# nerfstudio-project/gsplat

Hardware: AMD Instinct MI355X
Metric: Mpixels/s fwd+bwd @1M Gaussians/1080p (higher is better)
Workload: dtype f32; 1 GPU; c3: 1M synthetic Gaussians, 1x1920x1080, SH deg 3, 16x16 tiles, fwd+bwd; gaussians_per_gpu=1000000, cameras_per_gpu=1, packed=False, parallelism=single

## Files before the change

gsplat_amd/csrc/bitonic64.hpp:

```cpp
#pragma once
#include "common.hpp"

namespace gsx {

constexpr uint64_t kBtPadInt = ~0ull;
constexpr uint64_t kBtPadF64 = 0x7FF0000000000000ull;

__device__ __forceinline__ int bt_phys(int i) { return i + (i >> 3); }
__device__ __forceinline__ int bt_off(int b, int lj)
{
    const int sb = b << lj;
    return sb + (sb >> 3);
}
__device__ __forceinline__ bool bt_key_is_odd(uint32_t depth_bits)
{
    return (depth_bits - 0x00100000u) >= (0x7FF00000u - 0x00100000u);
}

__device__ __forceinline__ void bt_cmpx_int(uint64_t &x, uint64_t &y, bool up)
{
    const bool sw     = (x > y) == up;
    const uint64_t lo = sw ? y : x, hi = sw ? x : y;
    x = lo;
    y = hi;
}
__device__ __forceinline__ void bt_cmpx_int_up(uint64_t &x, uint64_t &y)
{
    const bool sw    = x > y;
    const uint64_t t = sw ? y : x;
    y                = sw ? x : y;
    x                = t;
}

template <int G, int NT>
__device__ __forceinline__ void bt_group_int(uint64_t *s, int P, int lk, int lj, int tid)
{
    constexpr int R = 1 << G;
    for (int t = tid; t < (P >> G); t += NT) {
        const int i = ((t >> lj) << (lj + G)) | (t & ((1 << lj) - 1));
        const uint32_t m32 = 0u - (((uint32_t)i >> lk) & 1u);
        const uint64_t m   = ((uint64_t)m32 << 32) | m32;
        uint64_t *p        = s + bt_phys(i);
        uint64_t e[R];
#pragma unroll
        for (int b = 0; b < R; ++b) e[b] = p[bt_off(b, lj)] ^ m;
#pragma unroll
        for (int q = G - 1; q >= 0; --q)
#pragma unroll
            for (int b = 0; b < R; ++b)
                if (!(b & (1 << q))) bt_cmpx_int_up(e[b], e[b | (1 << q)]);
#pragma unroll
        for (int b = 0; b < R; ++b) p[bt_off(b, lj)] = e[b] ^ m;
    }
}

template <int NT, typename Sync>
__device__ __forceinline__ void bt_sort_int(uint64_t *s, int lp, int tid, Sync &&SYNC)
{
    const int P = 1 << lp;
    for (int t = tid; t < (P >> 3); t += NT) {
        uint64_t *p = s + 9 * t;
        uint64_t e[8];
#pragma unroll
        for (int b = 0; b < 8; ++b) e[b] = p[b];
#pragma unroll
        for (int lk = 1; lk <= 3; ++lk)
#pragma unroll
            for (int q = lk - 1; q >= 0; --q)
#pragma unroll
                for (int b = 0; b < 8; ++b)
                    if (!(b & (1 << q))) {
                        const bool up = lk < 3 ? ((b & (1 << lk)) == 0) : ((t & 1) == 0);
                        bt_cmpx_int(e[b], e[b | (1 << q)], up);
                    }
#pragma unroll
        for (int b = 0; b < 8; ++b) p[b] = e[b];
    }
    SYNC();
    for (int lk = 4; lk <= lp; ++lk) {
        for (int top = lk - 1; top >= 0;) {
            const int gsz = top + 1 < 3 ? top + 1 : 3;
            const int lj  = top - gsz + 1;
            if (gsz == 3) bt_group_int<3, NT>(s, P, lk, lj, tid);
            else if (gsz == 2) bt_group_int<2, NT>(s, P, lk, lj, tid);
            else bt_group_int<1, NT>(s, P, lk, lj, tid);
            SYNC();
            top -= gsz;
        }
    }
}

__device__ __forceinline__ void bt_minmax(double &x, double &y)
{
    double lo, hi;
    asm("v_min_f64 %0, %1, %2" : "=v"(lo) : "v"(x), "v"(y));
    asm("v_max_f64 %0, %1, %2" : "=v"(hi) : "v"(x), "v"(y));
    x = lo;
    y = hi;
}
__device__ __forceinline__ double bt_as_f64(uint64_t w) { return __builtin_bit_cast(double, w); }
__device__ __forceinline__ uint64_t bt_as_u64(double d) { return __builtin_bit_cast(uint64_t, d); }

template <int G, int NT>
__device__ __forceinline__ void bt_group_f64(uint64_t *s, int P, int lk, int lj, int tid)
{
    constexpr int R = 1 << G;
    for (int t = tid; t < (P >> G); t += NT) {
        const int i = ((t >> lj) << (lj + G)) | (t & ((1 << lj) - 1));
        const uint64_t neg = (uint64_t)(((uint32_t)i >> lk) & 1u) << 63;
        uint64_t *p        = s + bt_phys(i);
        double e[R];
#pragma unroll
        for (int b = 0; b < R; ++b) e[b] = bt_as_f64(p[bt_off(b, lj)] ^ neg);
#pragma unroll
        for (int q = G - 1; q >= 0; --q)
#pragma unroll
            for (int b = 0; b < R; ++b)
                if (!(b & (1 << q))) bt_minmax(e[b], e[b | (1 << q)]);
#pragma unroll
        for (int b = 0; b < R; ++b) p[bt_off(b, lj)] = bt_as_u64(e[b]) ^ neg;
    }
}

template <int NT, typename Sync>
__device__ __forceinline__ void bt_sort_f64(uint64_t *s, int lp, int tid, Sync &&SYNC)
{
    const int P = 1 << lp;
    for (int t = tid; t < (P >> 3); t += NT) {
        uint64_t *p = s + 9 * t;
        double e[8];
#pragma unroll
        for (int b = 0; b < 8; ++b) e[b] = bt_as_f64(p[b]);
#pragma unroll
        for (int lk = 1; lk <= 2; ++lk)
#pragma unroll
            for (int q = lk - 1; q >= 0; --q)
#pragma unroll
                for (int b = 0; b < 8; ++b)
                    if (!(b & (1 << q))) {
                        if ((b & (1 << lk)) == 0) bt_minmax(e[b], e[b | (1 << q)]);
                        else bt_minmax(e[b | (1 << q)], e[b]);
                    }
        const uint64_t neg = (uint64_t)((uint32_t)t & 1u) << 63;
#pragma unroll
        for (int b = 0; b < 8; ++b) e[b] = bt_as_f64(bt_as_u64(e[b]) ^ neg);
#pragma unroll
        for (int q = 2; q >= 0; --q)
#pragma unroll
            for (int b = 0; b < 8; ++b)
                if (!(b & (1 << q))) bt_minmax(e[b], e[b | (1 << q)]);
#pragma unroll
        for (int b = 0; b < 8; ++b) p[b] = bt_as_u64(e[b]) ^ neg;
    }
    SYNC();
    for (int lk = 4; lk <= lp; ++lk) {
        for (int top = lk - 1; top >= 0;) {
            const int gsz = top + 1 < 3 ? top + 1 : 3;
            const int lj  = top - gsz + 1;
            if (gsz == 3) bt_group_f64<3, NT>(s, P, lk, lj, tid);
            else if (gsz == 2) bt_group_f64<2, NT>(s, P, lk, lj, tid);
            else bt_group_f64<1, NT>(s, P, lk, lj, tid);
            SYNC();
            top -= gsz;
        }
    }
}

bool bitonic_f64_enabled();

}
```

gsplat_amd/csrc/isect_binned.hip:

```cpp
#include "isect_binwalk.hpp"
#include "bitonic64.hpp"
#include "isect_fused.hpp"
#include <cstdlib>
#include <mutex>
#include <new>

namespace gsx {

constexpr int kRowThreads     = 1024;
constexpr int kBnThreads      = 256;
constexpr int kBnMaxBins      = 16384;
constexpr uint32_t kBnMaxTiles = 36864;

struct BinHeader {
    int32_t overflow;
    int32_t big_count;
    int32_t b_done;
    int32_t pad[5];
};

struct BinGeom {
    int64_t rows, rows_per_image, cap_entries;
    uint32_t n_images, cpi, rpc, n_chunks;
    uint32_t tile_size, tile_w, tile_h, n_tiles;
    uint32_t bw, bh, bins_x, bins_y, n_bins, n_bins_total, tile_bits;
    uint32_t kx, ky;
    int32_t skew_cap;
    int32_t skew_ratio;
};

struct BinBuffers {
    BinHeader *hdr;
    int32_t *table;
    int32_t *bin_count;
    int32_t *unit_count;
    uint4 *unit_rec;
    uint32_t *unit_row;
    int32_t *bin_start;
    uint4 *row_rec;
    uint2 *e_pair;
    uint16_t *e_mask;
    int32_t *tile_count;
    int32_t *big_list;
};

struct BinArgs {
    BinGeom g;
    BinBuffers b;
    const float *means2d;
    const int32_t *radii;
    const float *depths;
    const float *conics;
    const float *opacities;
    const uint8_t *tile_mask;
    int32_t *tiles_per_gauss;
    int32_t *isect_offsets;
    int64_t *n_isects;
    int64_t *max_tile_len;
    uint64_t *keys_out;
    int32_t *vals_out;
    uint2 *bucketed;
    uint32_t sort_int;
};

__device__ __forceinline__ void bn_chunk_rows(const BinGeom &g, uint32_t chunk, int64_t &lo, int64_t &hi, uint32_t &img)
{
    img                = chunk / g.cpi;
    const uint32_t sub = chunk % g.cpi;
    lo                 = (int64_t)img * g.rows_per_image + (int64_t)sub * g.rpc;
    hi                 = min(lo + (int64_t)g.rpc, (int64_t)(img + 1) * g.rows_per_image);
}

struct BnRow {
    float mx, my, rx, ry, A, B, C, op;
};
__device__ __forceinline__ BnRow bn_load_row(const BinArgs &a, int64_t r, bool has_conic)
{
    BnRow q;
    const int2 rad = reinterpret_cast<const int2 *>(a.radii)[r];
// ... 257 lines not shown
    int32_t v[kCsPer];
    int32_t sum = 0;
#pragma unroll
    for (int i = 0; i < kCsPer; ++i) {
        const uint32_t r = r0 + (uint32_t)i;
        v[i]             = (live && r < r1) ? col[(int64_t)r * n_cols] : 0;
    }
#pragma unroll
    for (int i = 0; i < kCsPer; ++i) sum += v[i];
    s_seg[seg][lane_c] = sum;
    __syncthreads();
    int32_t run = 0;
    for (uint32_t k = 0; k < seg; ++k) run += s_seg[k][lane_c];
    if (live) {
#pragma unroll
        for (int i = 0; i < kCsPer; ++i) {
            const uint32_t r = r0 + (uint32_t)i;
            if (r < r1) col[(int64_t)r * n_cols] = run;
            run += v[i];
        }
        if (seg == kCsSegs2 - 1) a.b.bin_count[(int64_t)img * n_cols + c] = run;
    }
    __syncthreads();
    if (threadIdx.x == 0)
        s_last = __hip_atomic_fetch_add(&a.b.hdr->b_done, 1, __ATOMIC_RELEASE, __HIP_MEMORY_SCOPE_AGENT) == (int32_t)gridDim.x - 1;
    __syncthreads();
    if (!s_last) return;
    __builtin_amdgcn_fence(__ATOMIC_ACQUIRE, "agent");
    const int64_t n = block_scan_i32_1024(a.b.bin_count, a.b.bin_start, g.n_bins_total, s_part, &s_max);
    int32_t um = 0;
    for (uint32_t i = threadIdx.x; i < g.n_chunks; i += kCsCols * kCsSegs2) um = max(um, a.b.unit_count[i]);
    um = wave_max_i32(um);
    if ((threadIdx.x & 63u) == 0) s_umax[threadIdx.x >> 6] = um;
    __syncthreads();
    if (threadIdx.x == 0) {
        for (int w = 1; w < 16; ++w) um = max(um, s_umax[w]);
        const int64_t mx    = s_max;
        const bool lopsided = g.skew_ratio > 0 && mx * (int64_t)g.n_bins_total > (int64_t)g.skew_ratio * n && mx > 256;
        a.b.bin_start[g.n_bins_total] = (int32_t)min(n, (int64_t)INT32_MAX);
        a.b.hdr->overflow = (n > g.cap_entries || um > (int32_t)kUnitCap || (g.skew_cap > 0 && mx > g.skew_cap) || lopsided) ? 1 : 0;
    }
}

template <bool FIXED>
__device__ __forceinline__ void bn_deal(const BinArgs &a, const BinShape<FIXED> &sh, const uint4 &rec, uint32_t row, int32_t *s_cur)
{
    const uint32_t bx0 = rec.z & 255u, by0 = (rec.z >> 8) & 255u;
    const uint64_t M   = ((uint64_t)rec.y << 32) | rec.x;
    for (uint32_t used = rec.z >> 18; used;) {
        const uint32_t k = (uint32_t)__builtin_ctz(used);
        used &= used - 1u;
        const uint32_t i = k % sh.kx, j = k / sh.kx;
        const int32_t slot = atomicAdd(&s_cur[(by0 + j) * a.g.bins_x + bx0 + i], 1);
        a.b.e_pair[slot] = make_uint2(rec.w, row);
        a.b.e_mask[slot] = (uint16_t)rec_bin_mask(M, sh, i, j);
    }
}

template <bool FIXED>
__global__ void __launch_bounds__(kRowThreads) bin_scatter_kernel(const BinArgs a)
{
    extern __shared__ int32_t s_cur[];
    const BinGeom &g = a.g;
    const BinShape<FIXED> sh(g);
    const uint32_t per_xcd = gridDim.x / 8u;
    const uint32_t chunk   = (blockIdx.x % 8u) * per_xcd + blockIdx.x / 8u;
    if (chunk >= g.n_chunks) return;
    int64_t lo, hi;
    uint32_t img;
    bn_chunk_rows(g, chunk, lo, hi, img);
    constexpr int kU = 2;
    uint4 rec[kU];
#pragma unroll
    for (int u = 0; u < kU; ++u) {
        const int64_t r = lo + u * kRowThreads + threadIdx.x;
        rec[u]          = r < hi ? a.b.row_rec[r] : make_uint4(0u, 0u, 0u, 0u);
    }
    const int32_t *start = a.b.bin_start + (int64_t)img * g.n_bins;
    const int32_t *pre   = a.b.table + (int64_t)chunk * g.n_bins;
    for (uint32_t i = threadIdx.x; i < g.n_bins; i += kRowThreads) s_cur[i] = start[i] + pre[i];
    const int32_t n_units = min(a.b.unit_count[chunk], (int32_t)kUnitCap);
    if (a.b.hdr->overflow) return;
    __syncthreads();
    for (int64_t base = lo; base < hi; base += kU * kRowThreads) {
#pragma unroll
        for (int u = 0; u < kU; ++u) {
            const int64_t r = base + u * kRowThreads + threadIdx.x;
            if (base != lo) rec[u] = r < hi ? a.b.row_rec[r] : make_uint4(0u, 0u, 0u, 0u);
            if (((rec[u].z >> 16) & 3u) == kRecSmall) bn_deal(a, sh, rec[u], (uint32_t)r, s_cur);
        }
    }
    for (int32_t k = (int32_t)threadIdx.x; k < n_units; k += kRowThreads)
        bn_deal(a, sh, a.b.unit_rec[(size_t)chunk * kUnitCap + k], a.b.unit_row[(size_t)chunk * kUnitCap + k], s_cur);
}

__global__ void __launch_bounds__(kBnThreads) bin_tiles_kernel(const BinArgs a)
{
    __shared__ int32_t s_cnt[16];
    const BinGeom &g = a.g;
    if (a.b.hdr->overflow) return;
    const uint32_t bin = blockIdx.x;
    const int32_t e0 = a.b.bin_start[bin], e1 = a.b.bin_start[bin + 1];
    const int lane = (int)(threadIdx.x & 63u);
    const int n_bits = (int)(g.bw * g.bh);
    if (threadIdx.x < 16) s_cnt[threadIdx.x] = 0;
    __syncthreads();
    int32_t mine = 0;
    constexpr int kU = 8;
    for (int32_t base = e0; base < e1; base += kBnThreads * kU) {
        uint32_t m[kU];
#pragma unroll
        for (int u = 0; u < kU; ++u) {
            const int32_t e = base + u * kBnThreads + (int32_t)threadIdx.x;
            m[u]            = e < e1 ? (uint32_t)a.b.e_mask[e] : 0u;
        }
#pragma unroll
        for (int u = 0; u < kU; ++u) {
            if (base + u * kBnThreads >= e1) break;
            for (int t = 0; t < n_bits; ++t) {
                const uint64_t b = __builtin_amdgcn_ballot_w64((m[u] >> t) & 1u);
                if (lane == t) mine += (int32_t)__popcll(b);
            }
        }
    }
    if (lane < n_bits && mine) atomicAdd(&s_cnt[lane], mine);
    __syncthreads();
    if ((int)threadIdx.x < n_bits) {
        const uint32_t img = bin / g.n_bins, lb = bin % g.n_bins;
        const uint32_t tx = (lb % g.bins_x) * g.bw + threadIdx.x % g.bw, ty = (lb / g.bins_x) * g.bh + threadIdx.x / g.bw;
        if (tx < g.tile_w && ty < g.tile_h) a.b.tile_count[(size_t)img * g.n_tiles + (size_t)ty * g.tile_w + tx] = s_cnt[threadIdx.x];
    }
}

__global__ void __launch_bounds__(1024) tile_plan_kernel(const BinArgs a)
{
    __shared__ int64_t s_part[16];
    __shared__ int32_t s_max;
    const BinGeom &g = a.g;
    if (a.b.hdr->overflow) {
        if (threadIdx.x == 0) {
            __threadfence_system();
            *a.n_isects = GSX_ISECT_RETRY;
        }
        return;
    }
    const uint32_t nt   = g.n_images * g.n_tiles;
    const int64_t total = block_scan_i32_1024(a.b.tile_count, a.isect_offsets, nt, s_part, a.max_tile_len ? &s_max : nullptr);
    if (threadIdx.x == 0) {
        if (a.max_tile_len) *a.max_tile_len = (int64_t)s_max;
        __threadfence_system();
        *a.n_isects = total;
    }
}

constexpr int kArenaPerWave = 544;

__host__ __device__ __forceinline__ int bn_list_words(int n, int &head)
{
    head = 0;
    if (n <= 0) return 0;
    int P = 64;
    while (P < n) P <<= 1;
    const int H = P >> 1;
    if (H >= 256 && n - H <= (H >> 2)) {
        head = H;
        return H + ((n - H + 7) & ~7);
    }
// ... 34 lines not shown
        } else {
            for (int i = lane; i < Pt; i += 64) {
                const uint64_t tv = sw[bt_phys(i)];
                sw[bt_phys(i)]    = keys[i];
                if (i < T) sw[bt_phys(H + i)] = tv;
            }
            lp = 31 - __builtin_clz((unsigned)H);
        }
        wave_lds_sync();
        if (as_int) bt_sort_int<64>(sw, lp, lane, [] { wave_lds_sync(); });
        else bt_sort_f64<64>(sw, lp, lane, [] { wave_lds_sync(); });
    }
    if (H == 0) {
        for (int i = lane; i < n; i += 64) {
            const uint64_t w = sw[bt_phys(i)];
            keys[i]          = hi | (w >> 32);
            vals[i]          = (int32_t)(uint32_t)w;
        }
        return;
    }
    for (int i0 = 0; i0 < H; i0 += 256) {
        uint64_t w[4];
        int r[4];
#pragma unroll
        for (int k = 0; k < 4; ++k) w[k] = sw[bt_phys(i0 + 64 * k + lane)];
        bn_rank4(sw, H, T, w, r);
#pragma unroll
        for (int k = 0; k < 4; ++k) {
            const int pos = i0 + 64 * k + lane + r[k];
            keys[pos]     = hi | (w[k] >> 32);
            vals[pos]     = (int32_t)(uint32_t)w[k];
        }
    }
    for (int j0 = 0; j0 < T; j0 += 256) {
        uint64_t w[4];
        int r[4];
#pragma unroll
        for (int k = 0; k < 4; ++k) {
            const int j = j0 + 64 * k + lane;
            w[k]        = j < T ? sw[bt_phys(H + j)] : 0ull;
        }
        bn_rank4(sw, 0, H, w, r);
#pragma unroll
        for (int k = 0; k < 4; ++k) {
            const int j = j0 + 64 * k + lane;
            if (j < T) {
                keys[j + r[k]] = hi | (w[k] >> 32);
                vals[j + r[k]] = (int32_t)(uint32_t)w[k];
            }
        }
    }
}

__global__ void __launch_bounds__(1024) __attribute__((amdgpu_waves_per_eu(8, 8))) bin_sort_kernel(const BinArgs a)
{
    extern __shared__ __attribute__((aligned(16))) unsigned char smem_raw[];
    const BinGeom &g = a.g;
    const int n_bits = (int)(g.bw * g.bh), n_thr = n_bits * 64;
    const int arena_words = kArenaPerWave * n_bits;
    uint64_t *s_arena = reinterpret_cast<uint64_t *>(smem_raw);
    __shared__ int32_t s_tcnt[16], s_goff[16], s_base[16], s_batch[16], s_cur[16], s_nbatch, s_n;
    __shared__ uint32_t s_odd;
    __shared__ uint64_t s_hi[16];
    const uint32_t bin = blockIdx.x;
    const int32_t e0 = a.b.bin_start[bin], e1 = a.b.bin_start[bin + 1];
    if (e0 == e1) return;
    const uint32_t img = bin / g.n_bins, lb = bin % g.n_bins;
    const uint32_t tx0 = (lb % g.bins_x) * g.bw, ty0 = (lb / g.bins_x) * g.bh;
    const int lane = (int)(threadIdx.x & 63u);
    const int wave = __builtin_amdgcn_readfirstlane((int)(threadIdx.x >> 6));
    if ((int)threadIdx.x < 16) {
        const int t       = (int)threadIdx.x;
        const uint32_t tx = tx0 + (uint32_t)t % g.bw, ty = ty0 + (uint32_t)t / g.bw;
        const bool in     = t < n_bits && tx < g.tile_w && ty < g.tile_h;
        const size_t gid  = (size_t)img * g.n_tiles + (size_t)ty * g.tile_w + tx;
        const int n       = in ? a.b.tile_count[gid] : 0;
        s_tcnt[t]         = n;
        s_goff[t]         = in ? a.isect_offsets[gid] : 0;
        s_hi[t]           = in ? ((((uint64_t)img << g.tile_bits) | ((uint64_t)ty * g.tile_w + tx)) << 32) : 0ull;
        int head;
        int P = bn_list_words(n, head);
        const bool big = P > arena_words;
        if (big) P = 0;
        int batch = 0, used = 0, my_batch = n > 0 ? 0 : -1, my_base = 0;
        for (int k = 0; k < 16; ++k) {
            const int Pk = __shfl(P, k, 16);
            if (Pk == 0) continue;
            if (used + Pk > arena_words) { ++batch; used = 0; }
            if (k == t) { my_batch = batch; my_base = used + (used >> 3); }
            used += Pk;
        }
        s_batch[t] = big ? -2 : my_batch;
        s_base[t]  = my_base;
        if (t == 15) s_nbatch = batch + 1;
    }
    __syncthreads();
    const int n_batch = s_nbatch;
    for (int b = 0; b < n_batch; ++b) {
        if (threadIdx.x < 16) s_cur[threadIdx.x] = 0;
        if (threadIdx.x == 16) s_odd = a.sort_int ? 0xFFFFu : 0u;
        const uint32_t bmask = (uint32_t)__builtin_amdgcn_ballot_w64(lane < n_bits && s_batch[lane & 15] == b);
        __syncthreads();
        for (int32_t e = e0 + (int32_t)threadIdx.x; e < e1; e += n_thr) {
            uint32_t m = (uint32_t)a.b.e_mask[e] & bmask;
            if (m == 0u) continue;
            const uint2 pr     = a.b.e_pair[e];
            const uint64_t key = ((uint64_t)pr.x << 32) | pr.y;
            if (bt_key_is_odd(pr.x)) atomicOr(&s_odd, m);
            while (m) {
                const int t = __builtin_ctz(m);
                m &= m - 1u;
                const int32_t pos = atomicAdd(&s_cur[t], 1);
                s_arena[s_base[t] + bt_phys(pos)] = key;
            }
        }
        __syncthreads();
        if (wave < n_bits && s_batch[wave] == b) {
            uint64_t *sw = s_arena + __builtin_amdgcn_readfirstlane(s_base[wave]);
            const int n  = __builtin_amdgcn_readfirstlane(s_tcnt[wave]);
            const bool as_int = (__builtin_amdgcn_readfirstlane((int)s_odd) >> wave) & 1;
            const int64_t off = __builtin_amdgcn_readfirstlane(s_goff[wave]);
            const uint64_t hi = (uint64_t)(uint32_t)__builtin_amdgcn_readfirstlane((int)(s_hi[wave] >> 32)) << 32;
            int head;
            bn_list_words(n, head);
            bn_sort_list(sw, n, head, as_int, lane, a.keys_out + off, a.vals_out + off, hi);
        }
        __syncthreads();
    }
    for (int t = 0; t < n_bits; ++t) {
        if (s_batch[t] != -2) continue;
        if (threadIdx.x == 0) s_n = 0;
        __syncthreads();
        const int64_t off      = s_goff[t];
        const uint64_t lt_mask = (lane == 0) ? 0ull : (~0ull >> (64 - lane));
        for (int32_t base = e0; base < e1; base += n_thr) {
            const int32_t e    = base + (int32_t)threadIdx.x;
            const bool has     = e < e1 && (((uint32_t)a.b.e_mask[e] >> t) & 1u);
            const uint64_t bal = __builtin_amdgcn_ballot_w64(has);
            if (bal == 0ull) continue;
            const int first = (int)__builtin_ctzll(bal);
            int32_t wbase   = 0;
            if (lane == first) wbase = atomicAdd(&s_n, (int32_t)__popcll(bal));
            wbase = __builtin_amdgcn_readlane(wbase, first);
            if (has) a.bucketed[off + wbase + (int32_t)__popcll(bal & lt_mask)] = a.b.e_pair[e];
        }
        if (threadIdx.x == 0) {
            const uint32_t tx = tx0 + (uint32_t)t % g.bw, ty = ty0 + (uint32_t)t / g.bw;
            a.b.big_list[atomicAdd(&a.b.hdr->big_count, 1)] = (int32_t)(img * g.n_tiles + ty * g.tile_w + tx);
        }
        __syncthreads();
    }
}

static int64_t align256(int64_t x) { return (x + 255) & ~(int64_t)255; }
static uint32_t bits_for(uint64_t count)
{
    uint32_t b = 0;
    if (count <= 1) return 0;
    uint64_t v = count - 1;
    while (v) { ++b; v >>= 1; }
    return b;
}

static void bin_dims(uint32_t &bw, uint32_t &bh)
{
    bw = 4; bh = 2;
    if (const char *e = getenv("GSX_ISECT_BIN")) {
        unsigned w = 0, h = 0;
        if (sscanf(e, "%ux%u", &w, &h) == 2 && w >= 1 && h >= 1 && w * h <= 16) { bw = w; bh = h; }
    }
}

static bool bin_geometry(BinGeom &g, int64_t rows, uint32_t n_images, uint32_t tile_size, uint32_t tile_w, uint32_t tile_h,
                         int64_t cap_entries)
{
    g = BinGeom{};
    g.rows = rows; g.n_images = n_images ? n_images : 1;
    g.rows_per_image = rows / g.n_images;
    bin_dims(g.bw, g.bh);
    g.tile_size = tile_size; g.tile_w = tile_w; g.tile_h = tile_h; g.n_tiles = tile_w * tile_h;
    g.bins_x = (tile_w + g.bw - 1) / g.bw; g.bins_y = (tile_h + g.bh - 1) / g.bh;
    g.kx = 2; g.ky = g.bw * g.bh <= 8 ? 4 : 2;
    g.n_bins = g.bins_x * g.bins_y; g.n_bins_total = g.n_bins * g.n_images;
    g.tile_bits = bits_for(g.n_tiles);
    const int64_t max_cpi = 1024 / g.n_images > 0 ? 1024 / g.n_images : 1;
    int64_t cpi = (g.rows_per_image + 2047) / 2048;
    {
        const int64_t per_image = (256 + (int64_t)g.n_images - 1) / (int64_t)g.n_images;
        const int64_t floor_cpi = g.rows_per_image / 1024 < per_image ? g.rows_per_image / 1024 : per_image;
        if (cpi < floor_cpi) cpi = floor_cpi;
    }
    if (cpi < 1) cpi = 1;
    if (cpi > max_cpi) cpi = max_cpi;
    g.cpi = (uint32_t)cpi;
    g.rpc = (uint32_t)((g.rows_per_image + cpi - 1) / cpi);
    if (g.rpc == 0) g.rpc = 1;
    g.n_chunks    = g.cpi * g.n_images;
    g.cap_entries = cap_entries;
    return g.n_bins_total <= (uint32_t)kBnMaxBins && (uint64_t)g.n_images * g.n_tiles <= kBnMaxTiles && rows < (1ll << 28)
           && g.bins_x <= 256 && g.bins_y <= 256;
}

static int64_t bin_cap_entries(int64_t rows) { return 4 * rows + 262144; }

static int64_t bin_layout(const BinGeom &g, unsigned char *base, BinBuffers *b)
{
    unsigned char *p = base;
    auto take = [&](int64_t bytes) {
        unsigned char *q = p;
        p += align256(bytes);
        return q;
    };
    BinBuffers t{};
    t.hdr        = reinterpret_cast<BinHeader *>(take(sizeof(BinHeader)));
    t.table      = reinterpret_cast<int32_t *>(take((int64_t)g.n_chunks * g.n_bins * 4));
    t.bin_count  = reinterpret_cast<int32_t *>(take((int64_t)g.n_bins_total * 4));
    t.unit_count = reinterpret_cast<int32_t *>(take((int64_t)g.n_chunks * 4));
    t.unit_rec   = reinterpret_cast<uint4 *>(take((int64_t)g.n_chunks * kUnitCap * 16));
    t.unit_row   = reinterpret_cast<uint32_t *>(take((int64_t)g.n_chunks * kUnitCap * 4));
    t.bin_start  = reinterpret_cast<int32_t *>(take(((int64_t)g.n_bins_total + 1) * 4));
    t.row_rec    = reinterpret_cast<uint4 *>(take(g.rows * 16));
    t.e_pair     = reinterpret_cast<uint2 *>(take(g.cap_entries * 8));
    t.e_mask     = reinterpret_cast<uint16_t *>(take(g.cap_entries * 2));
    t.tile_count = reinterpret_cast<int32_t *>(take((int64_t)g.n_images * g.n_tiles * 4));
    t.big_list   = reinterpret_cast<int32_t *>(take((int64_t)g.n_images * g.n_tiles * 4));
    if (b) *b = t;
    return (int64_t)(p - base);
}

}

using namespace gsx;

namespace {
struct RetryNote { uint64_t key; int left; };
struct PathMemory {
    std::mutex mu;
    RetryNote notes[16] = {};
    uint32_t next = 0;
};
thread_local PathMemory t_default_memory;
thread_local PathMemory *t_current_memory = nullptr;
PathMemory &current_memory() { return t_current_memory ? *t_current_memory : t_default_memory; }
uint64_t retry_key(int64_t rows, uint32_t n_images, uint32_t tile_w, uint32_t tile_h)
{
    return ((uint64_t)(rows >> 16) << 40) ^ ((uint64_t)n_images << 32) ^ ((uint64_t)tile_w << 16) ^ (uint64_t)tile_h ^ (1ull << 63);
}
bool retried_recently(int64_t rows, uint32_t n_images, uint32_t tile_w, uint32_t tile_h, bool consume)
{
    const uint64_t key = retry_key(rows, n_images, tile_w, tile_h);
    PathMemory &m = current_memory();
// ... 82 lines not shown
                "%s: %u images x %u x %u tiles not supported", fn, n_images, tile_w, tile_h);
    a.sort_int = bitonic_f64_enabled() ? 0u : 1u;
    {
        const char *force = getenv("GSX_ISECT_PATH");
        a.g.skew_cap = (force && force[0] == 'b') ? 0 : (int32_t)(kArenaPerWave * (int)(a.g.bw * a.g.bh) * 3 / 4);
        a.g.skew_ratio = (force && force[0] == 'b') ? 0 : 4;
    }
    unsigned char *base = reinterpret_cast<unsigned char *>((reinterpret_cast<uintptr_t>(ws) + 255) & ~(uintptr_t)255);
    if (ws == nullptr || (base - reinterpret_cast<unsigned char *>(ws)) + bin_layout(a.g, base, &a.b) > ws_bytes) {
        set_last_error("%s: count workspace too small", fn);
        return GSX_ERR_WORKSPACE;
    }
    return GSX_OK;
}

extern "C" int gsx_isect_binned_count(const float *means2d, const int32_t *radii, const float *depths, const float *conics,
                                      const float *opacities, const uint8_t *tile_mask, int64_t rows, uint32_t n_images,
                                      uint32_t tile_size, uint32_t tile_w, uint32_t tile_h, int32_t *tiles_per_gauss,
                                      int32_t *isect_offsets, int64_t *n_isects, int64_t *max_tile_len, void *count_workspace,
                                      int64_t count_workspace_bytes, void *stream)
{
    hipStream_t s = (hipStream_t)stream;
    const uint32_t n_bins = n_images * tile_w * tile_h;
    GSX_REQUIRE(isect_offsets && n_isects, "gsx_isect_binned_count: null output");
    if (rows == 0) {
        if (max_tile_len && hipMemsetAsync(max_tile_len, 0, 8, s) != hipSuccess) return check_launch("isect_binned_count memset");
        if (hipMemsetAsync(isect_offsets, 0, (size_t)n_bins * 4, s) != hipSuccess
            || hipMemsetAsync(n_isects, 0, 8, s) != hipSuccess) {
            set_last_error("gsx_isect_binned_count: memset failed");
            return GSX_ERR_LAUNCH;
        }
        return GSX_OK;
    }
    GSX_REQUIRE(means2d && radii && depths, "gsx_isect_binned_count: null pointer");
    BinArgs a{};
    int rc = binned_setup("gsx_isect_binned_count", a, rows, n_images, tile_size, tile_w, tile_h, count_workspace,
                          count_workspace_bytes);
    if (rc != GSX_OK) return rc;
    a.means2d = means2d; a.radii = radii; a.depths = depths; a.conics = conics; a.opacities = opacities;
    a.tile_mask = tile_mask; a.tiles_per_gauss = tiles_per_gauss; a.isect_offsets = isect_offsets; a.n_isects = n_isects;
    a.max_tile_len = max_tile_len;
    const size_t bins_lds = (size_t)a.g.n_bins * sizeof(int32_t);
    const bool fixed      = a.g.bw == 4 && a.g.bh == 2 && a.g.kx == 2 && a.g.ky == 4;
    static PerDeviceOnce once;
    if (once.first()) {
        (void)hipFuncSetAttribute((const void *)bin_rect_kernel<true>, hipFuncAttributeMaxDynamicSharedMemorySize, 64 * 1024);
        (void)hipFuncSetAttribute((const void *)bin_rect_kernel<false>, hipFuncAttributeMaxDynamicSharedMemorySize, 64 * 1024);
    }
    if (fixed) bin_rect_kernel<true><<<dim3(a.g.n_chunks), dim3(kRowThreads), bins_lds, s>>>(a);
    else bin_rect_kernel<false><<<dim3(a.g.n_chunks), dim3(kRowThreads), bins_lds, s>>>(a);
    const uint32_t col_groups = (a.g.n_bins + kCsCols - 1) / kCsCols;
    bin_colscan_kernel<<<dim3(col_groups * a.g.n_images), dim3(kCsCols * kCsSegs2), 0, s>>>(a, col_groups);
    const uint32_t d_grid = (a.g.n_chunks + 7u) / 8u * 8u;
    if (fixed) bin_scatter_kernel<true><<<dim3(d_grid), dim3(kRowThreads), bins_lds, s>>>(a);
    else bin_scatter_kernel<false><<<dim3(d_grid), dim3(kRowThreads), bins_lds, s>>>(a);
    bin_tiles_kernel<<<dim3(a.g.n_bins_total), dim3(kBnThreads), 0, s>>>(a);
    tile_plan_kernel<<<dim3(1), dim3(1024), 0, s>>>(a);
    return check_launch("isect_binned_count");
}

extern "C" int gsx_isect_binned_emit_sort(int64_t rows, uint32_t n_images, uint32_t tile_size, uint32_t tile_w,
                                          uint32_t tile_h, void *count_workspace, int64_t count_workspace_bytes,
                                          const int32_t *isect_offsets, int64_t n_isects, int64_t longest_list,
                                          int64_t *isect_ids_sorted, int32_t *flatten_ids_sorted, void *workspace,
                                          int64_t workspace_bytes, void *stream)
{
    GSX_REQUIRE(n_isects >= 0 && n_isects < (1ll << 31), "gsx_isect_binned_emit_sort: n_isects out of range");
    if (n_isects == 0 || rows == 0) return GSX_OK;
    GSX_REQUIRE(isect_offsets && isect_ids_sorted && flatten_ids_sorted, "gsx_isect_binned_emit_sort: null pointer");
    hipStream_t s = (hipStream_t)stream;
    BinArgs a{};
    int rc = binned_setup("gsx_isect_binned_emit_sort", a, rows, n_images, tile_size, tile_w, tile_h, count_workspace,
                          count_workspace_bytes);
    if (rc != GSX_OK) return rc;
    if (workspace == nullptr || workspace_bytes < gsx_isect_binned_emit_workspace_bytes(n_isects)) {
        set_last_error("gsx_isect_binned_emit_sort: workspace too small");
        return GSX_ERR_WORKSPACE;
    }
    unsigned char *p = reinterpret_cast<unsigned char *>((reinterpret_cast<uintptr_t>(workspace) + 255) & ~(uintptr_t)255);
    a.bucketed = reinterpret_cast<uint2 *>(p); p += align256(n_isects * 8);
    uint2 *scratch = reinterpret_cast<uint2 *>(p);
    a.isect_offsets = const_cast<int32_t *>(isect_offsets);
    a.keys_out = reinterpret_cast<uint64_t *>(isect_ids_sorted);
    a.vals_out = flatten_ids_sorted;
    const int n_bits = (int)(a.g.bw * a.g.bh);
    const size_t sort_lds = (size_t)(kArenaPerWave * n_bits) * 9;
    static PerDeviceOnce once;
    if (once.first())
        (void)hipFuncSetAttribute((const void *)bin_sort_kernel, hipFuncAttributeMaxDynamicSharedMemorySize, 112 * 1024);
    bin_sort_kernel<<<dim3(a.g.n_bins_total), dim3(64 * n_bits), sort_lds, s>>>(a);
    rc = check_launch("isect_binned_emit");
    if (rc != GSX_OK) return rc;
    TileSortArgs t{};
    t.n = n_isects; t.n_tiles = a.g.n_tiles; t.tile_bits = a.g.tile_bits; t.n_bins = a.g.n_images * a.g.n_tiles;
    t.n_chunks = 1;
    t.table_scanned = const_cast<int32_t *>(isect_offsets);
    t.bucketed = a.bucketed; t.scratch = scratch;
    t.big_count = &a.b.hdr->big_count; t.big_list = a.b.big_list;
    t.keys_out = a.keys_out; t.vals_out = a.vals_out;
    if (longest_list > 0 && longest_list <= (int64_t)(kArenaPerWave * n_bits) / 2) return GSX_OK;
    return launch_big_tile_sort(t, s);
}
```

gsplat_amd/csrc/isect_binwalk.hpp:

```cpp
#pragma once
#include "isect_walk.hpp"

namespace gsx {

struct WalkPrep {
    int x0, y0, x1, y1;
    bool any;
    bool ellipse, alongY;
    float B, coeff, disc, t, pu, pv, bmin_u, bmax_u, bmin_v, bmax_v, u_at_vmin, u_at_vmax;
};

__host__ __device__ __forceinline__ WalkPrep walk_prepare(float mx, float my, float rx, float ry, bool has_conic, float A,
                                                          float B, float C, float opacity, uint32_t tile_size,
                                                          uint32_t tile_w, uint32_t tile_h)
{
    WalkPrep p;
    p.any = false; p.ellipse = has_conic; p.alongY = false;
    p.x0 = p.y0 = p.x1 = p.y1 = 0;
    p.B = p.coeff = p.disc = p.t = p.pu = p.pv = p.bmin_u = p.bmax_u = p.bmin_v = p.bmax_v = p.u_at_vmin = p.u_at_vmax = 0.0f;
    const float ts     = (float)tile_size;
    const bool ts_pow2 = (tile_size & (tile_size - 1u)) == 0u;
    const float ts_inv = 1.0f / ts;
    auto div_ts        = [&](float x) { return ts_pow2 ? x * ts_inv : x / ts; };
    if (has_conic) {
// ... 84 lines not shown
        if (tv1 > cv1) tv1 = cv1;
        span(p.alongY, u, tv0, tv1);
        lo_lo   = hi_lo;
        lo_hi   = hi_hi;
        line_lo = line_hi;
    }
}

template <typename Emit>
__host__ __device__ __forceinline__ int32_t walk_clipped(const WalkPrep &p, uint32_t tile_size, int cx0, int cy0, int cx1,
                                                         int cy1, Emit &&emit)
{
    int32_t count = 0;
    walk_clipped_spans(p, tile_size, cx0, cy0, cx1, cy1, [&](bool alongY, int u, int tv0, int tv1) {
        for (int v = tv0; v < tv1; ++v) {
            if (alongY) emit(v, u);
            else emit(u, v);
            ++count;
        }
    });
    return count;
}

__host__ __device__ __forceinline__ uint64_t low_bits64(uint32_t n) { return n >= 64u ? ~0ull : ((1ull << n) - 1ull); }

__host__ __device__ __forceinline__ uint64_t block_mask(const WalkPrep &p, uint32_t tile_size, uint32_t tile_w, int cx0, int cy0,
                                                        int cx1, int cy1, uint32_t W, uint64_t col, const uint8_t *tmask)
{
    uint64_t M = 0;
    walk_clipped_spans(p, tile_size, cx0, cy0, cx1, cy1, [&](bool alongY, int uu, int tv0, int tv1) {
        if (tv1 <= tv0) return;
        if (alongY)
            M |= (low_bits64((uint32_t)(tv1 - cx0)) ^ low_bits64((uint32_t)(tv0 - cx0))) << ((uint32_t)(uu - cy0) * W);
        else
            M |= (col & (low_bits64((uint32_t)(tv1 - cy0) * W) ^ low_bits64((uint32_t)(tv0 - cy0) * W))) << (uu - cx0);
    });
    if (tmask)
        for (uint64_t left = M; left;) {
            const int b = __builtin_ctzll(left);
            left &= left - 1ull;
            if (!tmask[(size_t)(cy0 + b / (int)W) * tile_w + (size_t)(cx0 + b % (int)W)]) M &= ~(1ull << b);
        }
    return M;
}

__host__ __device__ __forceinline__ uint32_t block_bin_mask(uint64_t M, uint32_t bw, uint32_t bh, uint32_t kx, uint32_t i, uint32_t j)
{
    const uint32_t W = kx * bw, row_bits = (1u << bw) - 1u;
    uint32_t m = 0;
    for (uint32_t y = 0; y < bh; ++y) m |= ((uint32_t)(M >> ((j * bh + y) * W + i * bw)) & row_bits) << (y * bw);
    return m;
}

}
```

Baseline: 2633 Mpixels/s.

## Pack bin entries into one 64-bit word and sort each bin once

For the fixed 4x2-tile bin geometry, the scatter kernel now packs depth, per-image row and an 8-bit tile mask into one 64-bit word instead of writing separate pair and mask arrays. A new per-bin kernel loads a whole bin into LDS, bitonic-sorts it once, with per-wave sub-sorts followed by block-wide merge steps, and then deals the sorted entries out to the 8 tiles with ballots. This replaces the old path that re-gathered and sorted per tile. The old sort kernel still runs as a fallback for large bins, and the extra launch plus the 24-bit row limit add complexity.

```diff
diff --git a/gsplat_amd/csrc/bitonic64.hpp b/gsplat_amd/csrc/bitonic64.hpp
--- a/gsplat_amd/csrc/bitonic64.hpp
+++ b/gsplat_amd/csrc/bitonic64.hpp
@@ -33,11 +33,11 @@
 }
 
 template <int G, int NT>
-__device__ __forceinline__ void bt_group_int(uint64_t *s, int P, int lk, int lj, int tid)
+__device__ __forceinline__ void bt_group_int(uint64_t *s, int P, int lk, int lj, int tid, int ibase = 0)
 {
     constexpr int R = 1 << G;
     for (int t = tid; t < (P >> G); t += NT) {
-        const int i = ((t >> lj) << (lj + G)) | (t & ((1 << lj) - 1));
+        const int i = ibase + (((t >> lj) << (lj + G)) | (t & ((1 << lj) - 1)));
         const uint32_t m32 = 0u - (((uint32_t)i >> lk) & 1u);
         const uint64_t m   = ((uint64_t)m32 << 32) | m32;
         uint64_t *p        = s + bt_phys(i);
@@ -54,10 +54,9 @@
     }
 }
 
-template <int NT, typename Sync>
-__device__ __forceinline__ void bt_sort_int(uint64_t *s, int lp, int tid, Sync &&SYNC)
+template <int NT>
+__device__ __forceinline__ void bt_head_int(uint64_t *s, int P, int tid)
 {
-    const int P = 1 << lp;
     for (int t = tid; t < (P >> 3); t += NT) {
         uint64_t *p = s + 9 * t;
         uint64_t e[8];
@@ -76,18 +75,27 @@
 #pragma unroll
         for (int b = 0; b < 8; ++b) p[b] = e[b];
     }
+}
+template <int NT, typename Sync>
+__device__ __forceinline__ void bt_phase_int(uint64_t *s, int P, int lk, int top, int tid, int ibase, Sync &&SYNC)
+{
+    while (top >= 0) {
+        const int gsz = top + 1 < 3 ? top + 1 : 3;
+        const int lj  = top - gsz + 1;
+        if (gsz == 3) bt_group_int<3, NT>(s, P, lk, lj, tid, ibase);
+        else if (gsz == 2) bt_group_int<2, NT>(s, P, lk, lj, tid, ibase);
+        else bt_group_int<1, NT>(s, P, lk, lj, tid, ibase);
+        SYNC();
+        top -= gsz;
+    }
+}
+template <int NT, typename Sync>
+__device__ __forceinline__ void bt_sort_int(uint64_t *s, int lp, int tid, Sync &&SYNC)
+{
+    const int P = 1 << lp;
+    bt_head_int<NT>(s, P, tid);
     SYNC();
-    for (int lk = 4; lk <= lp; ++lk) {
-        for (int top = lk - 1; top >= 0;) {
-            const int gsz = top + 1 < 3 ? top + 1 : 3;
-            const int lj  = top - gsz + 1;
-            if (gsz == 3) bt_group_int<3, NT>(s, P, lk, lj, tid);
-            else if (gsz == 2) bt_group_int<2, NT>(s, P, lk, lj, tid);
-            else bt_group_int<1, NT>(s, P, lk, lj, tid);
-            SYNC();
-            top -= gsz;
-        }
-    }
+    for (int lk = 4; lk <= lp; ++lk) bt_phase_int<NT>(s, P, lk, lk - 1, tid, 0, SYNC);
 }
 
 __device__ __forceinline__ void bt_minmax(double &x, double &y)
@@ -102,11 +110,11 @@
 __device__ __forceinline__ uint64_t bt_as_u64(double d) { return __builtin_bit_cast(uint64_t, d); }
 
 template <int G, int NT>
-__device__ __forceinline__ void bt_group_f64(uint64_t *s, int P, int lk, int lj, int tid)
+__device__ __forceinline__ void bt_group_f64(uint64_t *s, int P, int lk, int lj, int tid, int ibase = 0)
 {
     constexpr int R = 1 << G;
     for (int t = tid; t < (P >> G); t += NT) {
-        const int i = ((t >> lj) << (lj + G)) | (t & ((1 << lj) - 1));
+        const int i = ibase + (((t >> lj) << (lj + G)) | (t & ((1 << lj) - 1)));
         const uint64_t neg = (uint64_t)(((uint32_t)i >> lk) & 1u) << 63;
         uint64_t *p        = s + bt_phys(i);
         double e[R];
@@ -122,10 +130,9 @@
     }
 }
 
-template <int NT, typename Sync>
-__device__ __forceinline__ void bt_sort_f64(uint64_t *s, int lp, int tid, Sync &&SYNC)
+template <int NT>
+__device__ __forceinline__ void bt_head_f64(uint64_t *s, int P, int tid)
 {
-    const int P = 1 << lp;
     for (int t = tid; t < (P >> 3); t += NT) {
         uint64_t *p = s + 9 * t;
         double e[8];
@@ -152,18 +159,27 @@
 #pragma unroll
         for (int b = 0; b < 8; ++b) p[b] = bt_as_u64(e[b]) ^ neg;
     }
+}
+template <int NT, typename Sync>
+__device__ __forceinline__ void bt_phase_f64(uint64_t *s, int P, int lk, int top, int tid, int ibase, Sync &&SYNC)
+{
+    while (top >= 0) {
+        const int gsz = top + 1 < 3 ? top + 1 : 3;
+        const int lj  = top - gsz + 1;
+        if (gsz == 3) bt_group_f64<3, NT>(s, P, lk, lj, tid, ibase);
+        else if (gsz == 2) bt_group_f64<2, NT>(s, P, lk, lj, tid, ibase);
+        else bt_group_f64<1, NT>(s, P, lk, lj, tid, ibase);
+        SYNC();
+        top -= gsz;
+    }
+}
+template <int NT, typename Sync>
+__device__ __forceinline__ void bt_sort_f64(uint64_t *s, int lp, int tid, Sync &&SYNC)
+{
+    const int P = 1 << lp;
+    bt_head_f64<NT>(s, P, tid);
     SYNC();
-    for (int lk = 4; lk <= lp; ++lk) {
-        for (int top = lk - 1; top >= 0;) {
-            const int gsz = top + 1 < 3 ? top + 1 : 3;
-            const int lj  = top - gsz + 1;
-            if (gsz == 3) bt_group_f64<3, NT>(s, P, lk, lj, tid);
-            else if (gsz == 2) bt_group_f64<2, NT>(s, P, lk, lj, tid);
-            else bt_group_f64<1, NT>(s, P, lk, lj, tid);
-            SYNC();
-            top -= gsz;
-        }
-    }
+    for (int lk = 4; lk <= lp; ++lk) bt_phase_f64<NT>(s, P, lk, lk - 1, tid, 0, SYNC);
 }
 
 bool bitonic_f64_enabled();
diff --git a/gsplat_amd/csrc/isect_binned.hip b/gsplat_amd/csrc/isect_binned.hip
--- a/gsplat_amd/csrc/isect_binned.hip
+++ b/gsplat_amd/csrc/isect_binned.hip
@@ -25,6 +25,7 @@
     uint32_t tile_size, tile_w, tile_h, n_tiles;
     uint32_t bw, bh, bins_x, bins_y, n_bins, n_bins_total, tile_bits;
     uint32_t kx, ky;
+    uint32_t word;
     int32_t skew_cap;
     int32_t skew_ratio;
 };
@@ -388,8 +389,12 @@
         used &= used - 1u;
         const uint32_t i = k % sh.kx, j = k / sh.kx;
         const int32_t slot = atomicAdd(&s_cur[(by0 + j) * a.g.bins_x + bx0 + i], 1);
-        a.b.e_pair[slot] = make_uint2(rec.w, row);
-        a.b.e_mask[slot] = (uint16_t)rec_bin_mask(M, sh, i, j);
+        if (FIXED) {
+            reinterpret_cast<uint64_t *>(a.b.e_pair)[slot] = bin_entry_pack(rec.w, row, rec_bin_mask(M, sh, i, j));
+        } else {
+            a.b.e_pair[slot] = make_uint2(rec.w, row);
+            a.b.e_mask[slot] = (uint16_t)rec_bin_mask(M, sh, i, j);
+        }
     }
 }
 
@@ -416,6 +421,7 @@
     const int32_t *pre   = a.b.table + (int64_t)chunk * g.n_bins;
     for (uint32_t i = threadIdx.x; i < g.n_bins; i += kRowThreads) s_cur[i] = start[i] + pre[i];
     const int32_t n_units = min(a.b.unit_count[chunk], (int32_t)kUnitCap);
+    const uint32_t row0   = FIXED ? (uint32_t)((int64_t)img * g.rows_per_image) : 0u;
     if (a.b.hdr->overflow) return;
     __syncthreads();
     for (int64_t base = lo; base < hi; base += kU * kRowThreads) {
@@ -423,11 +429,11 @@
         for (int u = 0; u < kU; ++u) {
             const int64_t r = base + u * kRowThreads + threadIdx.x;
             if (base != lo) rec[u] = r < hi ? a.b.row_rec[r] : make_uint4(0u, 0u, 0u, 0u);
-            if (((rec[u].z >> 16) & 3u) == kRecSmall) bn_deal(a, sh, rec[u], (uint32_t)r, s_cur);
+            if (((rec[u].z >> 16) & 3u) == kRecSmall) bn_deal(a, sh, rec[u], (uint32_t)r - row0, s_cur);
         }
     }
     for (int32_t k = (int32_t)threadIdx.x; k < n_units; k += kRowThreads)
-        bn_deal(a, sh, a.b.unit_rec[(size_t)chunk * kUnitCap + k], a.b.unit_row[(size_t)chunk * kUnitCap + k], s_cur);
+        bn_deal(a, sh, a.b.unit_rec[(size_t)chunk * kUnitCap + k], a.b.unit_row[(size_t)chunk * kUnitCap + k] - row0, s_cur);
 }
 
 __global__ void __launch_bounds__(kBnThreads) bin_tiles_kernel(const BinArgs a)
@@ -448,7 +454,7 @@
 #pragma unroll
         for (int u = 0; u < kU; ++u) {
             const int32_t e = base + u * kBnThreads + (int32_t)threadIdx.x;
-            m[u]            = e < e1 ? (uint32_t)a.b.e_mask[e] : 0u;
+            m[u]            = e >= e1 ? 0u : g.word ? bin_entry_mask(a.b.e_pair[e].x) : (uint32_t)a.b.e_mask[e];
         }
 #pragma unroll
         for (int u = 0; u < kU; ++u) {
@@ -589,6 +595,17 @@
     }
 }
 
+__device__ __forceinline__ uint64_t bn_entry_key(const BinArgs &a, int32_t e, uint32_t row0, uint32_t &mask)
+{
+    const uint2 pr = a.b.e_pair[e];
+    if (a.g.word) {
+        mask = bin_entry_mask(pr.x);
+        return ((uint64_t)pr.y << 32) | (bin_entry_row(pr.x) + row0);
+    }
+    mask = (uint32_t)a.b.e_mask[e];
+    return ((uint64_t)pr.x << 32) | pr.y;
+}
+
 __global__ void __launch_bounds__(1024) __attribute__((amdgpu_waves_per_eu(8, 8))) bin_sort_kernel(const BinArgs a)
 {
     extern __shared__ __attribute__((aligned(16))) unsigned char smem_raw[];
@@ -602,8 +619,10 @@
     const uint32_t bin = blockIdx.x;
     const int32_t e0 = a.b.bin_start[bin], e1 = a.b.bin_start[bin + 1];
     if (e0 == e1) return;
+    if (g.word && bin_sort_lp(e1 - e0)) return;
     const uint32_t img = bin / g.n_bins, lb = bin % g.n_bins;
     const uint32_t tx0 = (lb % g.bins_x) * g.bw, ty0 = (lb / g.bins_x) * g.bh;
+    const uint32_t row0 = g.word ? (uint32_t)((int64_t)img * g.rows_per_image) : 0u;
     const int lane = (int)(threadIdx.x & 63u);
     const int wave = __builtin_amdgcn_readfirstlane((int)(threadIdx.x >> 6));
     if ((int)threadIdx.x < 16) {
@@ -639,11 +658,11 @@
         const uint32_t bmask = (uint32_t)__builtin_amdgcn_ballot_w64(lane < n_bits && s_batch[lane & 15] == b);
         __syncthreads();
         for (int32_t e = e0 + (int32_t)threadIdx.x; e < e1; e += n_thr) {
-            uint32_t m = (uint32_t)a.b.e_mask[e] & bmask;
+            uint32_t m;
+            const uint64_t key = bn_entry_key(a, e, row0, m);
+            m &= bmask;
             if (m == 0u) continue;
-            const uint2 pr     = a.b.e_pair[e];
-            const uint64_t key = ((uint64_t)pr.x << 32) | pr.y;
-            if (bt_key_is_odd(pr.x)) atomicOr(&s_odd, m);
+            if (bt_key_is_odd((uint32_t)(key >> 32))) atomicOr(&s_odd, m);
             while (m) {
                 const int t = __builtin_ctz(m);
                 m &= m - 1u;
@@ -672,14 +691,16 @@
         const uint64_t lt_mask = (lane == 0) ? 0ull : (~0ull >> (64 - lane));
         for (int32_t base = e0; base < e1; base += n_thr) {
             const int32_t e    = base + (int32_t)threadIdx.x;
-            const bool has     = e < e1 && (((uint32_t)a.b.e_mask[e] >> t) & 1u);
+            uint32_t m         = 0u;
+            const uint64_t key = e < e1 ? bn_entry_key(a, e, row0, m) : 0ull;
+            const bool has     = (m >> t) & 1u;
             const uint64_t bal = __builtin_amdgcn_ballot_w64(has);
             if (bal == 0ull) continue;
             const int first = (int)__builtin_ctzll(bal);
             int32_t wbase   = 0;
             if (lane == first) wbase = atomicAdd(&s_n, (int32_t)__popcll(bal));
             wbase = __builtin_amdgcn_readlane(wbase, first);
-            if (has) a.bucketed[off + wbase + (int32_t)__popcll(bal & lt_mask)] = a.b.e_pair[e];
+            if (has) a.bucketed[off + wbase + (int32_t)__popcll(bal & lt_mask)] = make_uint2((uint32_t)(key >> 32), (uint32_t)key);
         }
         if (threadIdx.x == 0) {
             const uint32_t tx = tx0 + (uint32_t)t % g.bw, ty = ty0 + (uint32_t)t / g.bw;
@@ -687,6 +708,106 @@
         }
         __syncthreads();
     }
+}
+
+constexpr int kOnceThreads = 256;
+
+template <bool AS_INT>
+__device__ __forceinline__ void bn_sort_once(uint64_t *s, int lp, int wave, int lane)
+{
+    const int lr = lp - 2, R = 1 << lr, ibase = wave << lr;
+    auto fence   = [] { wave_lds_sync(); };
+    if (AS_INT) bt_head_int<64>(s + bt_phys(ibase), R, lane);
+    else bt_head_f64<64>(s + bt_phys(ibase), R, lane);
+    wave_lds_sync();
+    for (int lk = 4; lk <= lr; ++lk) {
+        if (AS_INT) bt_phase_int<64>(s, R, lk, lk - 1, lane, ibase, fence);
+        else bt_phase_f64<64>(s, R, lk, lk - 1, lane, ibase, fence);
+    }
+    for (int lk = lr + 1; lk <= lp; ++lk) {
+        __syncthreads();
+        const int tid = (int)threadIdx.x;
+        if (lk == lr + 1) {
+            if (AS_INT) bt_group_int<1, kOnceThreads>(s, 1 << lp, lk, lr, tid);
+            else bt_group_f64<1, kOnceThreads>(s, 1 << lp, lk, lr, tid);
+        } else {
+            if (AS_INT) bt_group_int<2, kOnceThreads>(s, 1 << lp, lk, lr, tid);
+            else bt_group_f64<2, kOnceThreads>(s, 1 << lp, lk, lr, tid);
+        }
+        __syncthreads();
+        if (AS_INT) bt_phase_int<64>(s, R, lk, lr - 1, lane, ibase, fence);
+        else bt_phase_f64<64>(s, R, lk, lr - 1, lane, ibase, fence);
+    }
+}
+
+__global__ void __launch_bounds__(kOnceThreads) __attribute__((amdgpu_waves_per_eu(8, 8))) bin_sort_once_kernel(const BinArgs a)
+{
+    __shared__ __attribute__((aligned(16))) uint64_t s_w[kBinSortMax + kBinSortMax / 8];
+    const BinGeom &g   = a.g;
+    const uint32_t bin = blockIdx.x;
+    const int32_t e0   = a.b.bin_start[bin];
+    const int n        = a.b.bin_start[bin + 1] - e0;
+    const int lp       = bin_sort_lp(n);
+    if (n == 0 || lp == 0) return;
+    const int P    = 1 << lp;
+    const int lane = (int)(threadIdx.x & 63u);
+    const int wave = __builtin_amdgcn_readfirstlane((int)(threadIdx.x >> 6));
+    const uint64_t *src = reinterpret_cast<const uint64_t *>(a.b.e_pair) + e0;
+    bool odd = a.sort_int != 0u;
+    for (int i = (int)threadIdx.x; i < n; i += kOnceThreads) {
+        const uint64_t w = src[i];
+        odd |= bt_key_is_odd(bin_entry_depth(w));
+        s_w[bt_phys(i)] = w;
+    }
+    const bool as_int  = __syncthreads_or(odd);
+    const uint64_t pad = as_int ? kBtPadInt : kBtPadF64;
+    for (int i = n + (int)threadIdx.x; i < P; i += kOnceThreads) s_w[bt_phys(i)] = pad;
+    __syncthreads();
+    if (as_int) bn_sort_once<true>(s_w, lp, wave, lane);
+    else bn_sort_once<false>(s_w, lp, wave, lane);
+    __syncthreads();
+    const uint32_t img = bin / g.n_bins, lb = bin % g.n_bins;
+    const uint32_t row0 = (uint32_t)((int64_t)img * g.rows_per_image);
+    const uint32_t ty0 = (lb / g.bins_x) * 2u, tx = (lb % g.bins_x) * 4u + (uint32_t)wave;
+    const uint64_t below = (1ull << lane) - 1ull;
+    uint64_t hi[2];
+    int64_t at[2];
+    uint32_t bit[2];
+#pragma unroll
+    for (int k = 0; k < 2; ++k) {
+        const uint32_t ty  = ty0 + (uint32_t)k;
+        const bool in      = tx < g.tile_w && ty < g.tile_h;
+        const uint32_t tid = in ? ty * g.tile_w + tx : 0u;
+        bit[k] = in ? 1u << (wave + 4 * k) : 0u;
+        at[k]  = a.isect_offsets[(size_t)img * g.n_tiles + tid];
+        hi[k]  = (((uint64_t)img << g.tile_bits) | tid) << 32;
+    }
+#ifdef GSX_ISECT_DBG
+    const int64_t at0[2] = {at[0], at[1]};
+#endif
+    for (int i0 = 0; i0 < n; i0 += 64) {
+        const int i      = i0 + lane;
+        const uint64_t w = i < n ? s_w[bt_phys(i)] : 0ull;
+        const uint32_t m = i < n ? bin_entry_mask(w) : 0u;
+#pragma unroll
+        for (int k = 0; k < 2; ++k) {
+            const bool has     = (m & bit[k]) != 0u;
+            const uint64_t bal = __builtin_amdgcn_ballot_w64(has);
+            if (has) {
+                const int64_t pos = at[k] + (int64_t)__popcll(bal & below);
+                a.keys_out[pos]   = hi[k] | bin_entry_depth(w);
+                a.vals_out[pos]   = (int32_t)(bin_entry_row(w) + row0);
+            }
+            at[k] += (int64_t)__popcll(bal);
+        }
+    }
+#ifdef GSX_ISECT_DBG
+    for (int k = 0; k < 2; ++k)
+        if (lane == 0 && bit[k]
+            && at[k] - at0[k] != a.b.tile_count[(size_t)img * g.n_tiles + (ty0 + (uint32_t)k) * g.tile_w + tx])
+            printf("bin_sort_once: bin %u tile bit %d: %lld entries, counted %d\n", bin, wave + 4 * k, (long long)(at[k] - at0[k]),
+                   a.b.tile_count[(size_t)img * g.n_tiles + (ty0 + (uint32_t)k) * g.tile_w + tx]);
+#endif
 }
 
 static int64_t align256(int64_t x) { return (x + 255) & ~(int64_t)255; }
@@ -734,6 +855,7 @@
     if (g.rpc == 0) g.rpc = 1;
     g.n_chunks    = g.cpi * g.n_images;
     g.cap_entries = cap_entries;
+    g.word = g.bw == 4 && g.bh == 2 && g.kx == 2 && g.ky == 4 && bin_entry_rows_ok(g.rows_per_image);
     return g.n_bins_total <= (uint32_t)kBnMaxBins && (uint64_t)g.n_images * g.n_tiles <= kBnMaxTiles && rows < (1ll << 28)
            && g.bins_x <= 256 && g.bins_y <= 256;
 }
@@ -922,7 +1044,7 @@
     const uint32_t col_groups = (a.g.n_bins + kCsCols - 1) / kCsCols;
     bin_colscan_kernel<<<dim3(col_groups * a.g.n_images), dim3(kCsCols * kCsSegs2), 0, s>>>(a, col_groups);
     const uint32_t d_grid = (a.g.n_chunks + 7u) / 8u * 8u;
-    if (fixed) bin_scatter_kernel<true><<<dim3(d_grid), dim3(kRowThreads), bins_lds, s>>>(a);
+    if (a.g.word) bin_scatter_kernel<true><<<dim3(d_grid), dim3(kRowThreads), bins_lds, s>>>(a);
     else bin_scatter_kernel<false><<<dim3(d_grid), dim3(kRowThreads), bins_lds, s>>>(a);
     bin_tiles_kernel<<<dim3(a.g.n_bins_total), dim3(kBnThreads), 0, s>>>(a);
     tile_plan_kernel<<<dim3(1), dim3(1024), 0, s>>>(a);
@@ -958,7 +1080,9 @@
     static PerDeviceOnce once;
     if (once.first())
         (void)hipFuncSetAttribute((const void *)bin_sort_kernel, hipFuncAttributeMaxDynamicSharedMemorySize, 112 * 1024);
-    bin_sort_kernel<<<dim3(a.g.n_bins_total), dim3(64 * n_bits), sort_lds, s>>>(a);
+    if (a.g.word) bin_sort_once_kernel<<<dim3(a.g.n_bins_total), dim3(kOnceThreads), 0, s>>>(a);
+    if (!(a.g.word && longest_list > 0 && 8 * longest_list <= (int64_t)kBinSortMax))
+        bin_sort_kernel<<<dim3(a.g.n_bins_total), dim3(64 * n_bits), sort_lds, s>>>(a);
     rc = check_launch("isect_binned_emit");
     if (rc != GSX_OK) return rc;
     TileSortArgs t{};
diff --git a/gsplat_amd/csrc/isect_binwalk.hpp b/gsplat_amd/csrc/isect_binwalk.hpp
--- a/gsplat_amd/csrc/isect_binwalk.hpp
+++ b/gsplat_amd/csrc/isect_binwalk.hpp
@@ -160,4 +160,23 @@
     return m;
 }
 
+constexpr uint32_t kBinEntryRowBits = 24;
+__host__ __device__ __forceinline__ bool bin_entry_rows_ok(int64_t rows_per_image) { return rows_per_image <= (1ll << kBinEntryRowBits); }
+__host__ __device__ __forceinline__ uint64_t bin_entry_pack(uint32_t depth_bits, uint32_t row_in_image, uint32_t mask)
+{
+    return ((uint64_t)depth_bits << 32) | ((uint64_t)row_in_image << 8) | (uint64_t)(mask & 0xFFu);
 }
+__host__ __device__ __forceinline__ uint32_t bin_entry_depth(uint64_t w) { return (uint32_t)(w >> 32); }
+__host__ __device__ __forceinline__ uint32_t bin_entry_row(uint64_t w) { return (uint32_t)w >> 8; }
+__host__ __device__ __forceinline__ uint32_t bin_entry_mask(uint64_t w) { return (uint32_t)w & 0xFFu; }
+
+constexpr int kBinSortMinLp = 8, kBinSortMaxLp = 11, kBinSortMax = 1 << kBinSortMaxLp;
+__host__ __device__ __forceinline__ int bin_sort_lp(int n)
+{
+    if (n > kBinSortMax) return 0;
+    int lp = kBinSortMinLp;
+    while ((1 << lp) < n) ++lp;
+    return lp;
+}
+
+}
```

Result: faster. 2691 Mpixels/s (median of 6 runs) (+2.2%).
